# NVlabs/STEP

Hardware: AMD Instinct MI355X
Metric: clips_per_sec_T32_224 (higher is better)
Workload: dtype bf16; 1 GPU; C2: I3D backbone (BaseNet conv3d_1a..mixed_4f) forward, 8 x [3,32,224,224] clips per GPU, inputs resident in HBM, random-init weights; clips_per_gpu=8, T=32, HW=224, parallelism=clip-sharded replicas x1 (no data-path collective), batches_in_flight=2

## Files before the change

step_amd/csrc/common.h:

```cpp
#pragma once
#include <stdint.h>
#include <float.h>
#include <math.h>

#ifdef STEP_EMUL
#include "hipemu.h"
#define STEP_WAVES_PER_SIMD(n)
#define STEP_WAVES_PER_SIMD_MIN(n)
#define STEP_SCHED_BARRIER()
#else
#include <hip/hip_runtime.h>
#define STEP_WAVES_PER_SIMD(n) __attribute__((amdgpu_waves_per_eu(n, n)))
#define STEP_WAVES_PER_SIMD_MIN(n) __attribute__((amdgpu_waves_per_eu(n)))
#define STEP_SCHED_BARRIER() __builtin_amdgcn_sched_barrier(0)
#endif

#include "../../include/step_amd.h"

namespace step {

typedef unsigned short u16x8 __attribute__((ext_vector_type(8)));
typedef unsigned short u16x4 __attribute__((ext_vector_type(4)));
typedef float f32x16 __attribute__((ext_vector_type(16)));
typedef float f32x8 __attribute__((ext_vector_type(8)));
typedef float f32x4 __attribute__((ext_vector_type(4)));
typedef float f32x2 __attribute__((ext_vector_type(2)));
typedef unsigned int u32x4 __attribute__((ext_vector_type(4)));

struct bf16_t { unsigned short v; };
struct f16_t { unsigned short v; };

__device__ __forceinline__ float bf16_bits_to_f32(unsigned short h) {
    unsigned int u = ((unsigned int)h) << 16;
    return __builtin_bit_cast(float, u);
}
__device__ __forceinline__ unsigned short f32_to_bf16_bits(float f) {
#ifndef STEP_EMUL
    return __builtin_bit_cast(unsigned short, (__bf16)f);
#endif
    unsigned int u = __builtin_bit_cast(unsigned int, f);
    if ((u & 0x7fffffffu) > 0x7f800000u) return (unsigned short)((u >> 16) | 0x40);
    u += 0x7fffu + ((u >> 16) & 1u);
    return (unsigned short)(u >> 16);
}
__device__ __forceinline__ float f16_bits_to_f32(unsigned short h) {
    _Float16 x = __builtin_bit_cast(_Float16, h);
    return (float)x;
}
__device__ __forceinline__ unsigned short f32_to_f16_bits(float f) {
    _Float16 x = (_Float16)f;
    return __builtin_bit_cast(unsigned short, x);
}

template <typename T> struct elem;
template <> struct elem<float> {
    static constexpr int dtype = STEP_F32;
    static constexpr int VEC = 4;
    __device__ static __forceinline__ float to_f32(float x) { return x; }
    __device__ static __forceinline__ float from_f32(float x) { return x; }
    __device__ static __forceinline__ unsigned short bits16(float) { return 0; }
    __device__ static __forceinline__ float from_bits16(unsigned short) { return 0.f; }
};
template <> struct elem<bf16_t> {
    static constexpr int dtype = STEP_BF16;
    static constexpr int VEC = 8;
    __device__ static __forceinline__ float to_f32(bf16_t x) { return bf16_bits_to_f32(x.v); }
    __device__ static __forceinline__ bf16_t from_f32(float x) { bf16_t r; r.v = f32_to_bf16_bits(x); return r; }
    __device__ static __forceinline__ unsigned short bits16(float x) { return f32_to_bf16_bits(x); }
    __device__ static __forceinline__ float from_bits16(unsigned short h) { return bf16_bits_to_f32(h); }
};
template <> struct elem<f16_t> {
    static constexpr int dtype = STEP_F16;
    static constexpr int VEC = 8;
    __device__ static __forceinline__ float to_f32(f16_t x) { return f16_bits_to_f32(x.v); }
    __device__ static __forceinline__ f16_t from_f32(float x) { f16_t r; r.v = f32_to_f16_bits(x); return r; }
    __device__ static __forceinline__ unsigned short bits16(float x) { return f32_to_f16_bits(x); }
    __device__ static __forceinline__ float from_bits16(unsigned short h) { return f16_bits_to_f32(h); }
};

template <typename T> struct frag;
template <> struct frag<float> { typedef f32x8 type; };
template <> struct frag<bf16_t> { typedef u16x8 type; };
template <> struct frag<f16_t> { typedef u16x8 type; };

#ifndef STEP_EMUL
typedef __bf16 bf16x8_hw __attribute__((ext_vector_type(8)));
typedef _Float16 f16x8_hw __attribute__((ext_vector_type(8)));
__device__ __forceinline__ void mma_k16(const f32x8& a, const f32x8& b, f32x16& c, float) {
#pragma unroll
    for (int j = 0; j < 8; ++j) c = __builtin_amdgcn_mfma_f32_32x32x2f32(a[j], b[j], c, 0, 0, 0);
}
__device__ __forceinline__ void mma_k16(const u16x8& a, const u16x8& b, f32x16& c, bf16_t) {
    c = __builtin_amdgcn_mfma_f32_32x32x16_bf16(__builtin_bit_cast(bf16x8_hw, a), __builtin_bit_cast(bf16x8_hw, b), c, 0, 0, 0);
}
__device__ __forceinline__ void mma_k16(const u16x8& a, const u16x8& b, f32x16& c, f16_t) {
    c = __builtin_amdgcn_mfma_f32_32x32x16_f16(__builtin_bit_cast(f16x8_hw, a), __builtin_bit_cast(f16x8_hw, b), c, 0, 0, 0);
}
#else
__device__ inline void mma_k16(const f32x8& a, const f32x8& b, f32x16& c, float) {
    float fa[8], fb[8];
    for (int j = 0; j < 8; ++j) { fa[j] = a[j]; fb[j] = b[j]; }
    hipemu::mfma_32x32_k16(fa, fb, c,  true);
}
__device__ inline void mma_k16(const u16x8& a, const u16x8& b, f32x16& c, bf16_t) {
    float fa[8], fb[8];
    for (int j = 0; j < 8; ++j) { fa[j] = bf16_bits_to_f32(a[j]); fb[j] = bf16_bits_to_f32(b[j]); }
    hipemu::mfma_32x32_k16(fa, fb, c, false);
}
__device__ inline void mma_k16(const u16x8& a, const u16x8& b, f32x16& c, f16_t) {
    float fa[8], fb[8];
    for (int j = 0; j < 8; ++j) { fa[j] = f16_bits_to_f32(a[j]); fb[j] = f16_bits_to_f32(b[j]); }
    hipemu::mfma_32x32_k16(fa, fb, c, false);
}
#endif

#ifndef STEP_EMUL
typedef short i16x4_hw __attribute__((ext_vector_type(4)));
__device__ __forceinline__ u16x8 lds_tr8(const unsigned char* a0, const unsigned char* a1) {
    typedef __attribute__((address_space(3))) i16x4_hw* lptr;
    const i16x4_hw lo = __builtin_amdgcn_ds_read_tr16_b64_v4i16((lptr)(const __attribute__((address_space(3))) unsigned char*)a0);
    const i16x4_hw hi = __builtin_amdgcn_ds_read_tr16_b64_v4i16((lptr)(const __attribute__((address_space(3))) unsigned char*)a1);
    u16x8 r = {(unsigned short)lo[0], (unsigned short)lo[1], (unsigned short)lo[2], (unsigned short)lo[3],
               (unsigned short)hi[0], (unsigned short)hi[1], (unsigned short)hi[2], (unsigned short)hi[3]};
    return r;
}
__device__ __forceinline__ void mma16_k32(const u16x8& a, const u16x8& b, f32x4& c, bf16_t) {
    c = __builtin_amdgcn_mfma_f32_16x16x32_bf16(__builtin_bit_cast(bf16x8_hw, a), __builtin_bit_cast(bf16x8_hw, b), c, 0, 0, 0);
}
__device__ __forceinline__ void mma16_k32(const u16x8& a, const u16x8& b, f32x4& c, f16_t) {
    c = __builtin_amdgcn_mfma_f32_16x16x32_f16(__builtin_bit_cast(f16x8_hw, a), __builtin_bit_cast(f16x8_hw, b), c, 0, 0, 0);
}
#else
__device__ inline u16x8 lds_tr8(const unsigned char* a0, const unsigned char* a1) {
    u16x8 r;
    for (int h = 0; h < 2; ++h) {
        unsigned short mine[4], out[4];
        __builtin_memcpy(mine, h ? a1 : a0, 8);
        hipemu::tr16_b64(mine, out);
        for (int j = 0; j < 4; ++j) r[h * 4 + j] = out[j];
    }
    return r;
}
__device__ inline void mma16_k32(const u16x8& a, const u16x8& b, f32x4& c, bf16_t) {
    float fa[8], fb[8];
    for (int j = 0; j < 8; ++j) { fa[j] = bf16_bits_to_f32(a[j]); fb[j] = bf16_bits_to_f32(b[j]); }
    hipemu::mfma_16x16_k32(fa, fb, c);
}
__device__ inline void mma16_k32(const u16x8& a, const u16x8& b, f32x4& c, f16_t) {
    float fa[8], fb[8];
    for (int j = 0; j < 8; ++j) { fa[j] = f16_bits_to_f32(a[j]); fb[j] = f16_bits_to_f32(b[j]); }
    hipemu::mfma_16x16_k32(fa, fb, c);
}
#endif

#ifndef STEP_EMUL
__device__ __forceinline__ void glds16(const void* gsrc_lane, void* lds_base_uniform) {
    __builtin_amdgcn_global_load_lds((const __attribute__((address_space(1))) void*)gsrc_lane,
                                     (__attribute__((address_space(3))) void*)lds_base_uniform, 16, 0, 0);
}
#else
__device__ inline void glds16(const void* gsrc_lane, void* lds_base_uniform) {
    __builtin_memcpy((unsigned char*)lds_base_uniform + 16 * (threadIdx.x & 63), gsrc_lane, 16);
}
#endif

__device__ __forceinline__ int cd_row(int r, int lane) { return (r & 3) + 8 * (r >> 2) + 4 * (lane >> 5); }

#ifndef STEP_EMUL
__device__ __forceinline__ void lane32_swap(unsigned& x, unsigned& y) {
    const auto r = __builtin_amdgcn_permlane32_swap(x, y, false, false);
    x = r[0]; y = r[1];
}
#else
__device__ inline void lane32_swap(unsigned& x, unsigned& y) {
    const unsigned mine[2] = {x, y};
    const int lane = (int)(threadIdx.x & 63);
    char* s = hipemu::exchange_begin(mine, 8);
    unsigned nx = x, ny = y;
    if (lane >= 32) __builtin_memcpy(&nx, s + 256 * (lane - 32) + 4, 4);
    else __builtin_memcpy(&ny, s + 256 * (lane + 32), 4);
    hipemu::exchange_end();
    x = nx; y = ny;
}
#endif

#ifdef STEP_EMUL
#define STEP_LAUNCH(kernel, grid, block, stream, ...) \
    hipemu::launch((grid), (block), [=]() { kernel(__VA_ARGS__); })
#define STEP_LAUNCH_CHECK() 0
#else
#define STEP_LAUNCH(kernel, grid, block, stream, ...) \
    hipLaunchKernelGGL(kernel, (grid), (block), 0, (hipStream_t)(stream), __VA_ARGS__)
#define STEP_LAUNCH_CHECK() ((int)hipGetLastError())
#endif

static inline int ceil_div(int a, int b) { return (a + b - 1) / b; }
static inline long long ceil_div64(long long a, long long b) { return (a + b - 1) / b; }

}
```

step_amd/csrc/stem.hip:

```cpp
#include "conv_common.h"

namespace step {

constexpr int STEM_TH = 8, STEM_TW = 16;
constexpr int STEM_ROWS = 2 * STEM_TH + 5, STEM_COLS = 40;

struct StemParams {
    const void* x; const void* w; const float* scale; const float* shift; void* y;
    int N, T, H, W, To, Ho, Wo, Cout, y_cstride, y_coff;
    int tiles_h, tiles_w, nblk32;
    int tile0;
    int relu;
    int Hp, Wp;
    void* rowbuf;
    void* colbuf;
    int u8_scale; float u8_mean[3], u8_std[3];
#ifdef STEP_PROBE
    unsigned long long* probe;
#endif
};

template <typename T, int NB>
__global__ __launch_bounds__(256) void stem_igemm_kernel(StemParams p) {
    constexpr int ES = (int)sizeof(T);
    constexpr int PIXB = 4 * ES;
    constexpr int NPIX = 7 * STEM_ROWS * STEM_COLS;
    typedef typename frag<T>::type frag_t;
    __shared__ __attribute__((aligned(16))) unsigned char lds[NPIX * PIXB];

    const int tid = threadIdx.x;
    const int lane = tid & 63, wave = tid >> 6;
    const int khalf = lane >> 5;
    const int m = wave * 32 + (lane & 31);
    const int th = m >> 4, tw = m & 15;

    int t = blockIdx.x;
    const int tw_i = t % p.tiles_w; t /= p.tiles_w;
    const int th_i = t % p.tiles_h; t /= p.tiles_h;
    const int od = t % p.To;
    const int n = t / p.To;
    const int oh0 = th_i * STEM_TH, ow0 = tw_i * STEM_TW;
    const int nb0 = blockIdx.y * NB;

    const T* xg = (const T*)p.x;
    const bool vec_ok = (p.W % 4) == 0;
    for (int item = tid; item < 7 * STEM_ROWS * (STEM_COLS / 4); item += 256) {
        const int cq = item % (STEM_COLS / 4);
        const int r = (item / (STEM_COLS / 4)) % STEM_ROWS;
        const int f = item / ((STEM_COLS / 4) * STEM_ROWS);
        const int it = 2 * od - 2 + f, ih = 2 * oh0 - 2 + r, iw0 = 2 * ow0 - 4 + cq * 4;
        T px[4][4];
#pragma unroll
        for (int a = 0; a < 4; ++a)
#pragma unroll
            for (int c = 0; c < 4; ++c) px[a][c] = elem<T>::from_f32(0.f);
        if (it >= 0 && it < p.T && ih >= 0 && ih < p.H) {
            const size_t base = (((size_t)n * p.T + it) * 3) * p.H * p.W + (size_t)ih * p.W;
#pragma unroll
            for (int c = 0; c < 3; ++c) {
                const T* src = xg + base + (size_t)c * p.H * p.W;
                if (vec_ok && iw0 >= 0 && iw0 + 3 < p.W) {
                    typedef unsigned int uvec __attribute__((ext_vector_type(ES)));
                    uvec raw = *(const uvec*)(src + iw0);
                    T v4[4];
                    __builtin_memcpy(v4, &raw, sizeof(v4));
#pragma unroll
                    for (int a = 0; a < 4; ++a) px[a][c] = v4[a];
                } else {
#pragma unroll
                    for (int a = 0; a < 4; ++a)
                        if (iw0 + a >= 0 && iw0 + a < p.W) px[a][c] = src[iw0 + a];
                }
            }
        }
        unsigned char* dst = lds + ((f * STEM_ROWS + r) * STEM_COLS + cq * 4) * PIXB;
#pragma unroll
        for (int q = 0; q < (4 * PIXB) / 16; ++q) {
            u32x4 tmp;
            __builtin_memcpy(&tmp, (const unsigned char*)&px[0][0] + 16 * q, 16);
            *(u32x4*)(dst + 16 * q) = tmp;
        }
    }
    __syncthreads();

    f32x16 acc[NB];
#pragma unroll
    for (int i = 0; i < NB; ++i)
#pragma unroll
        for (int r = 0; r < 16; ++r) acc[i][r] = 0.f;

    const T* wg = (const T*)p.w;
#pragma unroll 1
    for (int kd = 0; kd < 7; ++kd) {
#pragma unroll 1
        for (int kh = 0; kh < 7; ++kh) {
            const unsigned char* rowb = lds + ((kd * STEM_ROWS + 2 * th + kh) * STEM_COLS + 2 * tw + 2) * PIXB;
#pragma unroll
            for (int j = 0; j < 2; ++j) {
                const unsigned char* ap = rowb + (4 * j + 2 * khalf) * PIXB;
                frag_t a;
                {
                    u32x4 h2[ES / 2];
#pragma unroll
                    for (int q = 0; q < ES / 2; ++q) h2[q] = *(const u32x4*)(ap + 16 * q);
                    __builtin_memcpy(&a, h2, sizeof(a));
                }
                const int ks = (kd * 7 + kh) * 2 + j;
#pragma unroll
                for (int i = 0; i < NB; ++i) {
                    if (nb0 + i < p.nblk32) {
                        const T* bp = wg + (((size_t)(nb0 + i) * 98 + ks) * 64 + lane) * 8;
                        const frag_t b = load_b_frag<T>(bp);
                        mma_k16(a, b, acc[i], T());
                    }
                }
            }
        }
    }

    T* yg = (T*)p.y;
#pragma unroll
    for (int i = 0; i < NB; ++i) {
        const int co = (nb0 + i) * 32 + (lane & 31);
        if (nb0 + i < p.nblk32 && co < p.Cout) {
            const float sc = p.scale ? p.scale[co] : 1.f;
            const float sh = p.shift ? p.shift[co] : 0.f;
#pragma unroll
            for (int r = 0; r < 16; ++r) {
                const int mm = wave * 32 + cd_row(r, lane);
                const int oh = oh0 + (mm >> 4), ow = ow0 + (mm & 15);
                if (oh < p.Ho && ow < p.Wo) {
                    float v = acc[i][r] * sc + sh;
                    if (p.relu) v = fmaxf(v, 0.f);
                    const size_t opix = (((size_t)n * p.To + od) * p.Ho + oh) * p.Wo + ow;
                    yg[opix * p.y_cstride + p.y_coff + co] = elem<T>::from_f32(v);
                }
            }
        }
    }
}

constexpr int STP_ROWS = 37, STP_COLS = 40;

constexpr int STS_PITCH = 240;
constexpr int STS_FRAME = STP_ROWS * STS_PITCH;
constexpr int STS_KSTEPS = 77;

__device__ __forceinline__ u16x8 lds_read_frag_a4(const unsigned char* p) {
    typedef unsigned int u32x2_a4 __attribute__((ext_vector_type(2), aligned(4)));
    const u32x2_a4 lo = *(const u32x2_a4*)p;
    const u32x2_a4 hi = *(const u32x2_a4*)(p + 8);
    const u32x4 v = {lo.x, lo.y, hi.x, hi.y};
    u16x8 r;
    __builtin_memcpy(&r, &v, 16);
    return r;
}

constexpr int STS_TPITCH = 144;
typedef short s16x8_t __attribute__((ext_vector_type(8)));
__device__ __forceinline__ u32x4 pk_max_nonneg16(const u32x4& a, const u32x4& b) {
    return __builtin_bit_cast(u32x4, __builtin_elementwise_max(__builtin_bit_cast(s16x8_t, a), __builtin_bit_cast(s16x8_t, b)));
}

template <typename T, int NB_ = 2, bool VEC = true, bool POOL = false, bool U8 = false>
__global__ __launch_bounds__(256) STEP_WAVES_PER_SIMD(3) void stem_stream_kernel(StemParams p) {
    static_assert(sizeof(T) == 2, "16-bit storage types only");
    static_assert(!U8 || VEC, "uint8 frames: whole 4-column quads only");
    constexpr int FRAME = STS_FRAME, PITCH = STS_PITCH;
    constexpr int NB = NB_, FRAGB = 1024;
    constexpr int NBREG = 4 * FRAGB;
    constexpr int BBUF = NB * NBREG;
    constexpr int ITEMS = STP_ROWS * (STP_COLS / 4);
    constexpr int SL = 128;
    constexpr int FQ = (ITEMS + SL - 1) / SL;
    constexpr int NTILES = 21;
    typedef u16x8 frag_t;

    static_assert(!POOL || (NB == 2 && 256 * STS_TPITCH <= 3 * FRAME + 3 * BBUF), "the pooled epilogue's tile lives in the frame / weight rings");
    __shared__ __attribute__((aligned(16))) unsigned char lds[3 * FRAME + 3 * BBUF + NB * 32 * 2 * 4 + (U8 ? 3 * 256 * 2 : 0)];
    unsigned char* const ldsA = lds;
    unsigned char* const ldsB = lds + 3 * FRAME;
    float* const ldsS = (float*)(lds + 3 * FRAME + 3 * BBUF);
    unsigned short* const ldsL = (unsigned short*)(lds + 3 * FRAME + 3 * BBUF + NB * 32 * 2 * 4);

    const int tid = threadIdx.x;
    const int lane = tid & 63;
#ifdef STEP_EMUL
    const int wave = tid >> 6;
#else
    const int wave = __builtin_amdgcn_readfirstlane(tid >> 6);
#endif
    const int khalf = lane >> 5;
    const bool isW = wave < 2;
    const int stid = tid & (SL - 1);

    STEP_PROBE_IDS(p);
    STEP_PROBE_MARK(p, 0);
    int t = blockIdx.x;
    if ((gridDim.x & 7) == 0) t = (t & 7) * (gridDim.x >> 3) + (t >> 3);
    t += p.tile0;
    const int tw_i = t % p.tiles_w; t /= p.tiles_w;
    const int th_i = t % p.tiles_h; t /= p.tiles_h;
    const int od = t % p.To;
    const int n = t / p.To;
    const int oh0 = th_i * 16, ow0 = tw_i * 16;
    const int nb0 = blockIdx.y * NB;

    const T* xg = (const T*)p.x;
    const unsigned char* wg = (const unsigned char*)p.w;
    constexpr bool vec_ok = VEC;

    struct ItemP { u16x4 c[3]; };
    struct ItemB { unsigned w[3]; };
    typedef typename std::conditional<U8, ItemB, ItemP>::type Item;
    int qoff[FQ];
#pragma unroll
    for (int q = 0; q < FQ; ++q) {
        const int item = stid + q * SL;
        const int cq = item % (STP_COLS / 4), r = item / (STP_COLS / 4);
        const int ih = 2 * oh0 - 2 + r, iw0 = 2 * ow0 - 4 + cq * 4;
        qoff[q] = (item < ITEMS && ih >= 0 && ih < p.H && iw0 >= 0 && iw0 + 3 < p.W) ? ih * p.W + iw0 : -1;
    }
    const size_t plane_elems = (size_t)p.H * p.W;
    auto load_frame = [&](int f, Item (&it)[FQ]) {
        const int ifr = 2 * od - 2 + f;
        const bool frok = ifr >= 0 && ifr < p.T;
        const unsigned short* fbase = (const unsigned short*)xg + ((size_t)n * p.T + (frok ? ifr : 0)) * 3 * plane_elems;
        if constexpr (U8) {
            const unsigned char* fb8 = (const unsigned char*)p.x + ((size_t)n * p.T + (frok ? ifr : 0)) * 3 * plane_elems;
#pragma unroll
            for (int q = 0; q < FQ; ++q) {
                const unsigned* src = (const unsigned*)(fb8 + (size_t)(qoff[q] >= 0 ? qoff[q] : 0) * 3);
                it[q].w[0] = src[0]; it[q].w[1] = src[1]; it[q].w[2] = src[2];
            }
        } else if constexpr (vec_ok) {
#pragma unroll
            for (int q = 0; q < FQ; ++q) {
                const unsigned short* src = fbase + (qoff[q] >= 0 ? qoff[q] : 0);
#pragma unroll
                for (int c = 0; c < 3; ++c) it[q].c[c] = *(const u16x4*)(src + c * plane_elems);
            }
        } else {
#pragma unroll
        for (int q = 0; q < FQ; ++q) {
            const int item = stid + q * SL;
            const int cq = item % (STP_COLS / 4), r = item / (STP_COLS / 4);
            const int ih = 2 * oh0 - 2 + r, iw0 = 2 * ow0 - 4 + cq * 4;
            const bool rowok = item < ITEMS && frok && ih >= 0 && ih < p.H;
#pragma unroll
            for (int c = 0; c < 3; ++c) {
                u16x4 v = {0, 0, 0, 0};
                if (rowok) {
                    const unsigned short* src = fbase + c * plane_elems + (size_t)ih * p.W;
#pragma unroll
                    for (int a = 0; a < 4; ++a)
                        if (iw0 + a >= 0 && iw0 + a < p.W) v[a] = src[iw0 + a];
                }
                it[q].c[c] = v;
            }
        }
        }
    };
    auto store_frame = [&](int slotoff, int f, const Item (&it)[FQ]) {
        const int ifr = 2 * od - 2 + f;
        const bool frok = ifr >= 0 && ifr < p.T;
#pragma unroll
        for (int q = 0; q < FQ; ++q) {
            const int item = stid + q * SL;
            if (item < ITEMS) {
                const int cq = item % (STP_COLS / 4), r = item / (STP_COLS / 4);
                unsigned char* dst = ldsA + slotoff + r * PITCH + cq * 24;
                const unsigned short keep = (!vec_ok || (frok && qoff[q] >= 0)) ? 0xffffu : 0u;
                u16x4 v0, v1, v2;
                if constexpr (U8) {
                    unsigned short val[12];
#pragma unroll
                    for (int e = 0; e < 12; ++e) val[e] = ldsL[(e % 3) * 256 + ((it[q].w[e >> 2] >> (8 * (e & 3))) & 0xffu)];
                    v0 = u16x4{val[0], val[1], val[2], val[3]}; v1 = u16x4{val[4], val[5], val[6], val[7]}; v2 = u16x4{val[8], val[9], val[10], val[11]};
                } else {
                    v0 = u16x4{it[q].c[0][0], it[q].c[1][0], it[q].c[2][0], it[q].c[0][1]};
                    v1 = u16x4{it[q].c[1][1], it[q].c[2][1], it[q].c[0][2], it[q].c[1][2]};
                    v2 = u16x4{it[q].c[2][2], it[q].c[0][3], it[q].c[1][3], it[q].c[2][3]};
                }
#pragma unroll
                for (int e = 0; e < 4; ++e) { v0[e] &= keep; v1[e] &= keep; v2[e] &= keep; }
                *(u16x4*)dst = v0;
                *(u16x4*)(dst + 8) = v1;
                *(u16x4*)(dst + 16) = v2;
            }
        }
    };

    const unsigned char* wthr[NB];
#pragma unroll
    for (int i = 0; i < NB; ++i)
        wthr[i] = wg + ((size_t)min(nb0 + i, p.nblk32 - 1) * STS_KSTEPS) * FRAGB + stid * 16;
    struct BReg { u32x4 v[NB][2]; };
    auto load_B = [&](int tile) {
        tile = min(tile, NTILES - 1);
        const int ks0 = (tile / 3) * 11 + (tile % 3) * 4;
        BReg r;
#pragma unroll
        for (int i = 0; i < NB; ++i)
#pragma unroll
            for (int j = 0; j < 2; ++j) r.v[i][j] = *(const u32x4*)(wthr[i] + (size_t)ks0 * FRAGB + j * (SL * 16));
        return r;
    };
    auto store_B = [&](int buf, const BReg& r) {
#pragma unroll
        for (int i = 0; i < NB; ++i)
#pragma unroll
            for (int j = 0; j < 2; ++j) *(u32x4*)(ldsB + buf * BBUF + i * NBREG + j * (SL * 16) + stid * 16) = r.v[i][j];
    };

    const unsigned char* abase[2];
#pragma unroll
    for (int mb = 0; mb < 2; ++mb) {
        const int th = wave * 4 + mb + 2 * ((lane & 31) >> 4), tw = lane & 15;
        abase[mb] = ldsA + (2 * th) * PITCH + (2 * tw + 2) * 6;
    }
    const int kh_row = khalf * PITCH, kh_q = khalf * 16;
    const unsigned char* const bwave = ldsB + lane * 16;

    f32x16 acc[2][NB];
#pragma unroll
    for (int mb = 0; mb < 2; ++mb)
#pragma unroll
        for (int i = 0; i < NB; ++i)
#pragma unroll
            for (int r = 0; r < 16; ++r) acc[mb][i][r] = 0.f;

    frag_t fa[2][2], fb[2][NB];
    auto read_frags = [&](auto setc, auto jc, int slotoff) {
        constexpr int SET = decltype(setc)::value;
        constexpr int J = decltype(jc)::value;
        const int aoff = slotoff + (J < 9 ? (2 * (J / 3)) * PITCH + (J % 3) * 16 + kh_row : (J == 9 ? 6 * PITCH + kh_q : 6 * PITCH + 32));
#pragma unroll
        for (int mb = 0; mb < 2; ++mb) fa[SET][mb] = lds_read_frag_a4(abase[mb] + aoff);
#pragma unroll
        for (int i = 0; i < NB; ++i) fb[SET][i] = *(const frag_t*)(bwave + (J / 4) * BBUF + i * NBREG + (J % 4) * FRAGB);
    };
    auto mma_all = [&](auto setc) {
        constexpr int SET = decltype(setc)::value;
#pragma unroll
        for (int i = 0; i < NB; ++i) {
            mma_k16(fb[SET][i], fa[SET][0], acc[0][i], T());
            mma_k16(fb[SET][i], fa[SET][1], acc[1][i], T());
        }
    };

    if constexpr (U8) {
#pragma unroll
        for (int k = 0; k < 3; ++k) {
            float v = (float)tid;
            if (p.u8_scale == 1) v = __fdiv_rn(v, 255.f);
            else if (p.u8_scale == 2) v = __fsub_rn(__fdiv_rn(__fmul_rn(v, 2.f), 255.f), 1.f);
            v = __fdiv_rn(__fsub_rn(v, p.u8_mean[k]), p.u8_std[k]);
            ldsL[k * 256 + tid] = elem<T>::bits16(v);
        }
        __syncthreads();
    }
    auto run_role = [&](auto rolec) {
    constexpr bool W = decltype(rolec)::value;
    Item fr[FQ], fr1[FQ];
    Item frS[FQ];
    BReg R, R1;
    if constexpr (W) {
        float ss_sc = 1.f, ss_sh = 0.f;
        R = load_B(0);
        R1 = load_B(1);
        if (tid < NB * 32) {
            const int co = min(nb0 * 32 + tid, p.Cout - 1);
            if (p.scale) ss_sc = p.scale[co];
            if (p.shift) ss_sh = p.shift[co];
        }
        store_B(0, R);
        store_B(1, R1);
        if (tid < NB * 32) { ldsS[tid] = ss_sc; ldsS[NB * 32 + tid] = ss_sh; }
        R = load_B(2);
    } else {
        load_frame(0, fr);
        load_frame(1, fr1);
        load_frame(2, frS);
        store_frame(0, 0, fr);
        store_frame(FRAME, 1, fr1);
    }
    __syncthreads();
    STEP_PROBE_MARK(p, 1);
    read_frags(std::integral_constant<int, 0>(), std::integral_constant<int, 0>(), 0);

    int cur = 0, nxt = FRAME, nn = 2 * FRAME;
    auto frame_iter = [&](auto pc, auto ldc, auto stc, int kd) {
        constexpr int P = decltype(pc)::value;
        constexpr bool LD = decltype(ldc)::value, ST = decltype(stc)::value;
#define STS_KSTEP(J)                                                                                                  \
        {                                                                                                             \
            if (J < 10) read_frags(std::integral_constant<int, (P + J + 1) & 1>(), std::integral_constant<int, (J + 1) % 11>(), cur); \
            else        read_frags(std::integral_constant<int, (P + J + 1) & 1>(), std::integral_constant<int, 0>(), nxt);            \
            mma_all(std::integral_constant<int, (P + J) & 1>());                                                      \
        }
#define STS_TILE_END(TI)                                                                                              \
        {                                                                                                             \
            if constexpr (W) {                                                                                        \
                store_B((TI + 2) % 3, R);                                \
                R = load_B(3 * kd + TI + 3);                                                                          \
            }                                                                                                         \
        }
        STS_KSTEP(0) STS_KSTEP(1) STS_KSTEP(2) STS_KSTEP(3)
        STS_TILE_END(0)
        __syncthreads();
        STS_KSTEP(4) STS_KSTEP(5) STS_KSTEP(6) STS_KSTEP(7)
        STS_TILE_END(1)
        if constexpr (ST && !W) {
            STEP_SCHED_BARRIER();
            store_frame(nn, kd + 2, frS);
            if constexpr (LD) load_frame(kd + 3, frS);
        }
        __syncthreads();
        STS_KSTEP(8) STS_KSTEP(9) STS_KSTEP(10)
        STS_TILE_END(2)
        __syncthreads();
#undef STS_KSTEP
#undef STS_TILE_END
        const int tmp = cur; cur = nxt; nxt = nn; nn = tmp;
    };
#pragma unroll 1
    for (int kd = 0; kd < 4; kd += 2) {
        frame_iter(std::integral_constant<int, 0>(), std::true_type(), std::true_type(), kd);
        frame_iter(std::integral_constant<int, 1>(), std::true_type(), std::true_type(), kd + 1);
        STEP_PROBE_MARK(p, 5 + kd / 2);
    }
    frame_iter(std::integral_constant<int, 0>(), std::false_type(), std::true_type(), 4);
    frame_iter(std::integral_constant<int, 1>(), std::false_type(), std::false_type(), 5);
    STEP_PROBE_MARK(p, 7);
    frame_iter(std::integral_constant<int, 0>(), std::false_type(), std::false_type(), 6);
    };
    if (isW) run_role(std::true_type());
    else run_role(std::false_type());
    STEP_PROBE_MARK(p, 2);

    T* yg = (T*)p.y;
    const bool vec_epi = (p.y_cstride % 8 == 0) && (p.y_coff % 8 == 0) && (p.Cout % 8 == 0) && (((uintptr_t)p.y) % 16 == 0);
#pragma unroll
    for (int mb = 0; mb < 2; ++mb) {
        const int oh = oh0 + wave * 4 + mb + 2 * ((lane & 31) >> 4), ow = ow0 + (lane & 15);
        const bool okp = oh < p.Ho && ow < p.Wo;
        const size_t opix = okp ? (((size_t)n * p.To + od) * p.Ho + oh) * p.Wo + ow : 0;
#pragma unroll
        for (int i = 0; i < NB; ++i) {
            unsigned d[4][2];
#pragma unroll
            for (int g = 0; g < 4; ++g) {
                const f32x4 sc = *(const f32x4*)(ldsS + i * 32 + 8 * g + 4 * khalf);
                const f32x4 sh = *(const f32x4*)(ldsS + NB * 32 + i * 32 + 8 * g + 4 * khalf);
                float v[4];
#pragma unroll
                for (int e = 0; e < 4; ++e) {
                    v[e] = acc[mb][i][4 * g + e] * sc[e] + sh[e];
                    if (p.relu) v[e] = fmaxf(v[e], 0.f);
                }
                if (!vec_epi && !POOL) {
#pragma unroll
                    for (int e = 0; e < 4; ++e) {
                        const int co = (nb0 + i) * 32 + 8 * g + 4 * khalf + e;
                        if (okp && co < p.Cout) yg[opix * p.y_cstride + p.y_coff + co] = elem<T>::from_f32(v[e]);
                    }
                }
                d[g][0] = (unsigned)elem<T>::bits16(v[0]) | ((unsigned)elem<T>::bits16(v[1]) << 16);
                d[g][1] = (unsigned)elem<T>::bits16(v[2]) | ((unsigned)elem<T>::bits16(v[3]) << 16);
            }
            if constexpr (POOL) {
                const int tpix = (wave * 4 + mb + 2 * ((lane & 31) >> 4)) * 16 + (lane & 15);
#pragma unroll
                for (int h = 0; h < 2; ++h) {
                    lane32_swap(d[2 * h][0], d[2 * h + 1][0]);
                    lane32_swap(d[2 * h][1], d[2 * h + 1][1]);
                    u32x4 o = {d[2 * h][0], d[2 * h][1], d[2 * h + 1][0], d[2 * h + 1][1]};
                    if (!okp) o = u32x4{0u, 0u, 0u, 0u};
                    *(u32x4*)(lds + tpix * STS_TPITCH + (i * 32 + 16 * h + 8 * khalf) * 2) = o;
                }
            } else if (vec_epi) {
#pragma unroll
                for (int h = 0; h < 2; ++h) {
                    lane32_swap(d[2 * h][0], d[2 * h + 1][0]);
                    lane32_swap(d[2 * h][1], d[2 * h + 1][1]);
                    const int co = (nb0 + i) * 32 + 16 * h + 8 * khalf;
                    if (okp && co < p.Cout) {
                        const u32x4 o = {d[2 * h][0], d[2 * h][1], d[2 * h + 1][0], d[2 * h + 1][1]};
                        *(u32x4*)(yg + opix * p.y_cstride + p.y_coff + co) = o;
                    }
                }
            }
        }
    }
    if constexpr (POOL) {
        __syncthreads();
        const size_t plane = (size_t)n * p.To + od;
#pragma unroll
        for (int k = 0; k < 2; ++k) {
            const int item = tid + 256 * k;
            const int v = item & 7, q = (item >> 3) & 7, j = item >> 6;
            const unsigned char* base = lds + ((2 * j) * 16 + 2 * q) * STS_TPITCH + v * 16;
            u32x4 m = *(const u32x4*)base;
#pragma unroll
            for (int dr = 0; dr < 3; ++dr)
#pragma unroll
                for (int dc = 0; dc < 3; ++dc) {
                    if (dr == 0 && dc == 0) continue;
                    if (2 * j + dr < 16 && 2 * q + dc < 16) m = pk_max_nonneg16(m, *(const u32x4*)(base + (dr * 16 + dc) * STS_TPITCH));
                }
            const int ph = (oh0 >> 1) + j, pw = (ow0 >> 1) + q;
            if (ph < p.Hp && pw < p.Wp)
                *(u32x4*)(yg + ((plane * p.Hp + ph) * p.Wp + pw) * p.y_cstride + p.y_coff + v * 8) = m;
        }
        {
            const int v = tid & 7, e = (tid >> 3) & 15;
            unsigned short* rb = (unsigned short*)p.rowbuf;
            unsigned short* cb = (unsigned short*)p.colbuf;
            if (tid < 128) {
                if (th_i > 0 && ow0 + e < p.Wo)
                    *(u32x4*)(rb + ((plane * p.tiles_h + th_i) * p.Wo + ow0 + e) * (size_t)p.Cout + v * 8) = *(const u32x4*)(lds + e * STS_TPITCH + v * 16);
            } else {
                if (tw_i > 0 && oh0 + e < p.Ho)
                    *(u32x4*)(cb + ((plane * p.tiles_w + tw_i) * p.Ho + oh0 + e) * (size_t)p.Cout + v * 8) = *(const u32x4*)(lds + (e * 16) * STS_TPITCH + v * 16);
            }
        }
    }
#ifdef STEP_PROBE
    STEP_PROBE_MARK(p, 3);
    __builtin_amdgcn_s_waitcnt(0);
    probe_clock_end(p.probe);
    STEP_PROBE_MARK(p, 4);
#endif
}

__global__ __launch_bounds__(256) void stem_pool_fix_kernel(StemParams p) {
    const int nbr = p.tiles_h - 1, nbc = p.tiles_w - 1;
    const long long per_plane = ((long long)nbr * p.Wp + (long long)nbc * p.Hp) * (p.Cout / 8);
    const long long total = per_plane * p.N * p.To;
    const int V = p.Cout / 8;
    unsigned short* yg = (unsigned short*)p.y;
    const unsigned short* rb = (const unsigned short*)p.rowbuf;
    const unsigned short* cb = (const unsigned short*)p.colbuf;
    for (long long idx = (long long)blockIdx.x * blockDim.x + threadIdx.x; idx < total; idx += (long long)blockDim.x * gridDim.x) {
        const long long plane = idx / per_plane;
        long long it = idx % per_plane;
        const int v = (int)(it % V);
        it /= V;
        int ph, pw;
        bool row_item;
        if (it < (long long)nbr * p.Wp) { row_item = true; ph = 8 * ((int)(it / p.Wp) + 1) - 1; pw = (int)(it % p.Wp); }
        else { it -= (long long)nbr * p.Wp; row_item = false; pw = 8 * ((int)(it / p.Hp) + 1) - 1; ph = (int)(it % p.Hp); }
        if (ph >= p.Hp || pw >= p.Wp) continue;
        const bool ph_seam = ((ph + 1) & 7) == 0 && ((ph + 1) >> 3) <= nbr;
        const bool pw_seam = ((pw + 1) & 7) == 0 && ((pw + 1) >> 3) <= nbc;
        if (!row_item && ph_seam) continue;
        unsigned short* yp = yg + ((plane * p.Hp + ph) * p.Wp + pw) * (size_t)p.y_cstride + p.y_coff + v * 8;
        u32x4 m = *(const u32x4*)yp;
        if (row_item) {
            const int t = (ph + 1) >> 3;
            for (int dc = 0; dc < 3; ++dc) {
                const int c = 2 * pw + dc;
                if (c < p.Wo) m = pk_max_nonneg16(m, *(const u32x4*)(rb + ((plane * p.tiles_h + t) * p.Wo + c) * (size_t)p.Cout + v * 8));
            }
            if (pw_seam) {
                const int s = (pw + 1) >> 3;
                for (int dr = 0; dr < 2; ++dr)
                    m = pk_max_nonneg16(m, *(const u32x4*)(cb + ((plane * p.tiles_w + s) * p.Ho + 2 * ph + dr) * (size_t)p.Cout + v * 8));
            }
        } else {
            const int s = (pw + 1) >> 3;
            for (int dr = 0; dr < 3; ++dr) {
                const int r = 2 * ph + dr;
                if (r < p.Ho) m = pk_max_nonneg16(m, *(const u32x4*)(cb + ((plane * p.tiles_w + s) * p.Ho + r) * (size_t)p.Cout + v * 8));
            }
        }
        *(u32x4*)yp = m;
    }
}

template <typename T>
__global__ void stem_stream_pack_weight_kernel(const float* __restrict__ w, T* __restrict__ out, int Cout, long long total) {
    for (long long idx = (long long)blockIdx.x * blockDim.x + threadIdx.x; idx < total;
         idx += (long long)blockDim.x * gridDim.x) {
        const int e = (int)(idx & 7);
        const int lane = (int)((idx >> 3) & 63);
        const long long q = idx >> 9;
        const int ks = (int)(q % STS_KSTEPS);
        const long long nb = q / STS_KSTEPS;
        const int kd = ks / 11, j = ks % 11, khalf = lane >> 5;
        int kh, fq;
        if (j < 9) { kh = 2 * (j / 3) + khalf; fq = j % 3; }
        else if (j == 9) { kh = 6; fq = khalf; }
        else { kh = 6; fq = khalf ? -1 : 2; }
        const int se = 8 * fq + e, kw = se / 3, c = se % 3;
        const long long co = nb * 32 + (lane & 31);
        float v = 0.f;
        if (fq >= 0 && co < Cout && kw < 7) v = w[((((size_t)co * 3 + c) * 7 + kd) * 7 + kh) * 7 + kw];
        out[idx] = elem<T>::from_f32(v);
    }
}

template <typename T>
__global__ void stem_pack_weight_kernel(const float* __restrict__ w, T* __restrict__ out, int Cout, long long total) {
    for (long long idx = (long long)blockIdx.x * blockDim.x + threadIdx.x; idx < total;
         idx += (long long)blockDim.x * gridDim.x) {
        const int e = (int)(idx & 7);
        const int lane = (int)((idx >> 3) & 63);
        long long q = idx >> 9;
        const int ks = (int)(q % 98);
        const int nb = (int)(q / 98);
        const int j = ks & 1, kh = (ks >> 1) % 7, kd = (ks >> 1) / 7;
        const int kw = 4 * j + 2 * (lane >> 5) + (e >> 2), c = e & 3;
        const int co = nb * 32 + (lane & 31);
        float v = 0.f;
        if (co < Cout && c < 3 && kw < 7) v = w[((((size_t)co * 3 + c) * 7 + kd) * 7 + kh) * 7 + kw];
        out[idx] = elem<T>::from_f32(v);
    }
}


template <typename T>
static int stem_forward_t(StemParams p, step_stream_t stream) {
    dim3 grid((unsigned)((long long)p.N * p.To * p.tiles_h * p.tiles_w), (unsigned)ceil_div(p.nblk32, 2));
    STEP_LAUNCH((stem_igemm_kernel<T, 2>), grid, dim3(256), stream, p);
    return STEP_LAUNCH_CHECK();
}

static inline size_t stem_stream_offset(int Cout) { return (size_t)ceil_div(Cout, 32) * 98 * 512; }

template <typename T>
static int stem_stream_forward_t(StemParams p, step_stream_t stream) {
    p.w = (const T*)p.w + stem_stream_offset(p.Cout);
    p.tiles_h = ceil_div(p.Ho, 16); p.tiles_w = ceil_div(p.Wo, 16);
    const long long tiles = (long long)p.N * p.To * p.tiles_h * p.tiles_w;
    const int groups = ceil_div(p.nblk32, 2);
    p.tile0 = 0;
#ifdef STEP_PROBE
    p.probe = g_probe_buf;
#endif
    dim3 grid((unsigned)tiles, (unsigned)groups);
    if (p.W % 4 == 0) STEP_LAUNCH((stem_stream_kernel<T, 2, true>), grid, dim3(256), stream, p);
    else STEP_LAUNCH((stem_stream_kernel<T, 2, false>), grid, dim3(256), stream, p);
    return STEP_LAUNCH_CHECK();
}


}

using namespace step;

extern "C" {

size_t step_stem_packed_elems(int Cout) { return stem_stream_offset(Cout) + ((size_t)ceil_div(Cout, 32) * STS_KSTEPS + 1) * 512; }

int step_stem_pack_weight(const float* w, int Cout, int dtype, void* packed, step_stream_t stream) {
    if (Cout <= 0) return STEP_E_SHAPE;
    if (!w || !packed) return STEP_E_NULL;
    const long long total = (long long)stem_stream_offset(Cout);
    const long long total2 = (long long)step_stem_packed_elems(Cout) - total;
    const dim3 grid(flat_grid(total, 256)), grid2(flat_grid(total2, 256));
    switch (dtype) {
        case STEP_F32:
            STEP_LAUNCH((stem_pack_weight_kernel<float>), grid, dim3(256), stream, w, (float*)packed, Cout, total);
            STEP_LAUNCH((stem_stream_pack_weight_kernel<float>), grid2, dim3(256), stream, w, (float*)packed + total, Cout, total2);
            break;
        case STEP_BF16:
            STEP_LAUNCH((stem_pack_weight_kernel<bf16_t>), grid, dim3(256), stream, w, (bf16_t*)packed, Cout, total);
            STEP_LAUNCH((stem_stream_pack_weight_kernel<bf16_t>), grid2, dim3(256), stream, w, (bf16_t*)packed + total, Cout, total2);
            break;
        case STEP_F16:
            STEP_LAUNCH((stem_pack_weight_kernel<f16_t>), grid, dim3(256), stream, w, (f16_t*)packed, Cout, total);
            STEP_LAUNCH((stem_stream_pack_weight_kernel<f16_t>), grid2, dim3(256), stream, w, (f16_t*)packed + total, Cout, total2);
            break;
        default: return STEP_E_DTYPE;
    }
    return STEP_LAUNCH_CHECK();
}

int step_stem_forward(int dtype, const void* x, int N, int T, int H, int W, const void* w_packed, const float* scale,
                      const float* shift, int relu, int Cout, void* y, int y_cstride, int y_coff, step_stream_t stream) {
    if (N < 0 || T <= 0 || H <= 0 || W <= 0 || Cout <= 0) return STEP_E_SHAPE;
    if (y_coff < 0 || y_coff + Cout > y_cstride) return STEP_E_SHAPE;
    if (N == 0) return STEP_OK;
    if (!x || !w_packed || !y) return STEP_E_NULL;
    if (((uintptr_t)x % 16) || ((uintptr_t)w_packed % 16)) return STEP_E_ALIGN;
    StemParams p;
    p.x = x; p.w = w_packed; p.scale = scale; p.shift = shift; p.y = y;
    p.N = N; p.T = T; p.H = H; p.W = W; p.tile0 = 0; p.relu = relu != 0;
    p.To = (T + 5 - 7) / 2 + 1; p.Ho = (H + 5 - 7) / 2 + 1; p.Wo = (W + 5 - 7) / 2 + 1;
    if (p.To <= 0 || p.Ho <= 0 || p.Wo <= 0) return STEP_E_SHAPE;
    p.Cout = Cout; p.y_cstride = y_cstride; p.y_coff = y_coff;
    p.tiles_h = ceil_div(p.Ho, STEM_TH); p.tiles_w = ceil_div(p.Wo, STEM_TW);
    p.nblk32 = ceil_div(Cout, 32);
    const int ov = conv_impl_override();
    switch (dtype) {
        case STEP_F32: return stem_forward_t<float>(p, stream);
        case STEP_BF16: return ov == 0 ? stem_forward_t<bf16_t>(p, stream) : stem_stream_forward_t<bf16_t>(p, stream);
        case STEP_F16: return ov == 0 ? stem_forward_t<f16_t>(p, stream) : stem_stream_forward_t<f16_t>(p, stream);
    }
    return STEP_E_DTYPE;
}


static bool stem_pool_supported(int dtype, int N, int T, int H, int W, int Cout) {
    return (dtype == STEP_BF16 || dtype == STEP_F16) && N > 0 && T > 0 && H > 0 && W > 0 && (W % 4) == 0 && Cout == 64 && conv_impl_override() != 0;
}

size_t step_stem_pool_workspace_bytes(int dtype, int N, int T, int H, int W, int Cout) {
    if (!stem_pool_supported(dtype, N, T, H, W, Cout)) return 0;
    const int To = (T - 2) / 2 + 1, Ho = (H - 2) / 2 + 1, Wo = (W - 2) / 2 + 1;
    const size_t planes = (size_t)N * To;
    return planes * ((size_t)ceil_div(Ho, 16) * Wo + (size_t)ceil_div(Wo, 16) * Ho) * Cout * 2 + 32;
}

static int stem_pool_forward_impl(int dtype, const void* x, int N, int T, int H, int W, const void* w_packed, const float* scale, const float* shift,
                                  int Cout, void* y, int y_cstride, int y_coff, void* ws, size_t ws_bytes, int parts, step_stream_t stream) {
    if (N < 0 || T <= 0 || H <= 0 || W <= 0 || Cout <= 0) return STEP_E_SHAPE;
    if (y_coff < 0 || y_coff + Cout > y_cstride) return STEP_E_SHAPE;
    if (N == 0) return STEP_OK;
    if (!stem_pool_supported(dtype, N, T, H, W, Cout)) return STEP_E_UNSUPPORTED;
    if (!x || !w_packed || !y || !ws) return STEP_E_NULL;
    if (((uintptr_t)x % 16) || ((uintptr_t)w_packed % 16) || ((uintptr_t)y % 16) || ((uintptr_t)ws % 16) || (y_cstride % 8) || (y_coff % 8)) return STEP_E_ALIGN;
    if (ws_bytes < step_stem_pool_workspace_bytes(dtype, N, T, H, W, Cout)) return STEP_E_SHAPE;
    StemParams p;
    p.x = x; p.scale = scale; p.shift = shift; p.y = y;
    p.N = N; p.T = T; p.H = H; p.W = W; p.tile0 = 0; p.relu = 1;
    p.To = (T + 5 - 7) / 2 + 1; p.Ho = (H + 5 - 7) / 2 + 1; p.Wo = (W + 5 - 7) / 2 + 1;
    if (p.To <= 0 || p.Ho <= 0 || p.Wo <= 0) return STEP_E_SHAPE;
    p.Cout = Cout; p.y_cstride = y_cstride; p.y_coff = y_coff;
    p.nblk32 = ceil_div(Cout, 32);
    p.tiles_h = ceil_div(p.Ho, 16); p.tiles_w = ceil_div(p.Wo, 16);
    p.Hp = step_pool_out_size(p.Ho, 3, 2); p.Wp = step_pool_out_size(p.Wo, 3, 2);
    p.rowbuf = ws;
    p.colbuf = (unsigned char*)ws + (((size_t)N * p.To * p.tiles_h * p.Wo * Cout * 2 + 15) / 16) * 16;
#ifdef STEP_PROBE
    p.probe = g_probe_buf;
#endif
    const long long tiles = (long long)p.N * p.To * p.tiles_h * p.tiles_w;
    dim3 grid((unsigned)tiles, 1);
    if (parts & 1) {
        if (dtype == STEP_BF16) {
            p.w = (const bf16_t*)w_packed + stem_stream_offset(Cout);
            STEP_LAUNCH((stem_stream_kernel<bf16_t, 2, true, true>), grid, dim3(256), stream, p);
        } else {
            p.w = (const f16_t*)w_packed + stem_stream_offset(Cout);
            STEP_LAUNCH((stem_stream_kernel<f16_t, 2, true, true>), grid, dim3(256), stream, p);
        }
    }
    if ((parts & 2) && (p.tiles_h > 1 || p.tiles_w > 1)) {
        const long long items = ((long long)(p.tiles_h - 1) * p.Wp + (long long)(p.tiles_w - 1) * p.Hp) * (Cout / 8) * p.N * p.To;
        STEP_LAUNCH(stem_pool_fix_kernel, dim3(flat_grid(items, 256)), dim3(256), stream, p);
    }
    return STEP_LAUNCH_CHECK();
}

int step_stem_pool_forward(int dtype, const void* x, int N, int T, int H, int W, const void* w_packed, const float* scale, const float* shift,
                           int Cout, void* y, int y_cstride, int y_coff, void* ws, size_t ws_bytes, step_stream_t stream) {
    return stem_pool_forward_impl(dtype, x, N, T, H, W, w_packed, scale, shift, Cout, y, y_cstride, y_coff, ws, ws_bytes, 3, stream);
}

int step_stem_pool_forward_tiles(int dtype, const void* x, int N, int T, int H, int W, const void* w_packed, const float* scale, const float* shift,
                                 int Cout, void* y, int y_cstride, int y_coff, void* ws, size_t ws_bytes, step_stream_t stream) {
    return stem_pool_forward_impl(dtype, x, N, T, H, W, w_packed, scale, shift, Cout, y, y_cstride, y_coff, ws, ws_bytes, 1, stream);
}

int step_stem_pool_finish(int dtype, const void* x, int N, int T, int H, int W, int Cout, void* y, int y_cstride, int y_coff, void* ws, size_t ws_bytes,
                          step_stream_t stream) {
    return stem_pool_forward_impl(dtype, x, N, T, H, W, x, nullptr, nullptr, Cout, y, y_cstride, y_coff, ws, ws_bytes, 2, stream);
}

int step_stem_pool_forward_u8(int dtype, const unsigned char* frames, int N, int T, int H, int W, int u8_scale, const float* mean3, const float* std3,
                              const void* w_packed, const float* scale, const float* shift, int Cout, void* y, int y_cstride, int y_coff,
                              void* ws, size_t ws_bytes, step_stream_t stream) {
    if (N < 0 || T <= 0 || H <= 0 || W <= 0 || Cout <= 0 || u8_scale < 0 || u8_scale > 2) return STEP_E_SHAPE;
    if (y_coff < 0 || y_coff + Cout > y_cstride) return STEP_E_SHAPE;
    if (N == 0) return STEP_OK;
    if (!stem_pool_supported(dtype, N, T, H, W, Cout)) return STEP_E_UNSUPPORTED;
    if (!frames || !w_packed || !y || !ws) return STEP_E_NULL;
    if (((uintptr_t)frames % 4) || ((uintptr_t)w_packed % 16) || ((uintptr_t)y % 16) || ((uintptr_t)ws % 16) || (y_cstride % 8) || (y_coff % 8)) return STEP_E_ALIGN;
    if (ws_bytes < step_stem_pool_workspace_bytes(dtype, N, T, H, W, Cout)) return STEP_E_SHAPE;
    StemParams p;
    p.x = frames; p.scale = scale; p.shift = shift; p.y = y;
    p.N = N; p.T = T; p.H = H; p.W = W; p.tile0 = 0; p.relu = 1;
    p.To = (T + 5 - 7) / 2 + 1; p.Ho = (H + 5 - 7) / 2 + 1; p.Wo = (W + 5 - 7) / 2 + 1;
    if (p.To <= 0 || p.Ho <= 0 || p.Wo <= 0) return STEP_E_SHAPE;
    p.Cout = Cout; p.y_cstride = y_cstride; p.y_coff = y_coff;
    p.nblk32 = ceil_div(Cout, 32);
    p.tiles_h = ceil_div(p.Ho, 16); p.tiles_w = ceil_div(p.Wo, 16);
    p.Hp = step_pool_out_size(p.Ho, 3, 2); p.Wp = step_pool_out_size(p.Wo, 3, 2);
    p.rowbuf = ws;
    p.colbuf = (unsigned char*)ws + (((size_t)N * p.To * p.tiles_h * p.Wo * Cout * 2 + 15) / 16) * 16;
    p.u8_scale = u8_scale;
    for (int c = 0; c < 3; ++c) { p.u8_mean[c] = mean3 ? mean3[c] : 0.f; p.u8_std[c] = std3 ? std3[c] : 1.f; }
#ifdef STEP_PROBE
    p.probe = g_probe_buf;
#endif
    const long long tiles = (long long)p.N * p.To * p.tiles_h * p.tiles_w;
    dim3 grid((unsigned)tiles, 1);
    if (dtype == STEP_BF16) {
        p.w = (const bf16_t*)w_packed + stem_stream_offset(Cout);
        STEP_LAUNCH((stem_stream_kernel<bf16_t, 2, true, true, true>), grid, dim3(256), stream, p);
    } else {
        p.w = (const f16_t*)w_packed + stem_stream_offset(Cout);
        STEP_LAUNCH((stem_stream_kernel<f16_t, 2, true, true, true>), grid, dim3(256), stream, p);
    }
    if (p.tiles_h > 1 || p.tiles_w > 1) {
        const long long items = ((long long)(p.tiles_h - 1) * p.Wp + (long long)(p.tiles_w - 1) * p.Hp) * (Cout / 8) * p.N * p.To;
        STEP_LAUNCH(stem_pool_fix_kernel, dim3(flat_grid(items, 256)), dim3(256), stream, p);
    }
    return STEP_LAUNCH_CHECK();
}

int step_stem_kernel_name(int dtype, char* buf, int buflen) {
    if (!buf || buflen <= 0) return STEP_E_NULL;
    const int ov = conv_impl_override();
    const char* t = dtype == STEP_F32 ? "float" : (dtype == STEP_BF16 ? "step::bf16_t" : "step::f16_t");
    if (dtype != STEP_F32 && dtype != STEP_BF16 && dtype != STEP_F16) return STEP_E_DTYPE;
    if (dtype == STEP_F32 || ov == 0) snprintf(buf, (size_t)buflen, "void step::stem_igemm_kernel<%s, 2>(step::StemParams)", t);
    else snprintf(buf, (size_t)buflen, "void step::stem_stream_kernel<%s, 2, true, false, false>(step::StemParams)", t);
    return STEP_OK;
}


}
```

Before: 7552 clips/s.

## Stream stem weight tiles via direct global-to-LDS DMA with four-deep ring

The weight waves of the stem conv kernel now load weight fragments with global_load_lds straight into LDS instead of going through registers and storing them. Each tile shrinks from four k-steps to three, and the ring grows to four buffers, giving 28 tiles with a vmcnt-based wait. An extra barrier per frame separates the new fourth tile. The intent is to remove VGPR staging and LDS store instructions on the weight path and keep more weight loads in flight. In exchange it uses more LDS, adds one __syncthreads per frame, and relies on hand-written m0 asm whose vmcnt accounting must match exactly.

```diff
diff --git a/step_amd/csrc/common.h b/step_amd/csrc/common.h
--- a/step_amd/csrc/common.h
+++ b/step_amd/csrc/common.h
@@ -164,6 +164,19 @@
 }
 #endif
 
+#ifndef STEP_EMUL
+__device__ __forceinline__ void glds16_uncounted(const void* gsrc_lane, void* lds_base_uniform) {
+    const unsigned dst = __builtin_amdgcn_readfirstlane((unsigned)(uintptr_t)(__attribute__((address_space(3))) void*)lds_base_uniform);
+    unsigned keep;
+    asm volatile("s_mov_b32 %0, m0\n\ts_mov_b32 m0, %2\n\ts_nop 0\n\tglobal_load_lds_dwordx4 %1, off\n\ts_mov_b32 m0, %0"
+                 : "=&s"(keep) : "v"(gsrc_lane), "s"(dst) : "memory");
+}
+template <int N> __device__ __forceinline__ void vmcnt_wait() { asm volatile("s_waitcnt vmcnt(%0)" :: "i"(N) : "memory"); }
+#else
+__device__ inline void glds16_uncounted(const void* gsrc_lane, void* lds_base_uniform) { glds16(gsrc_lane, lds_base_uniform); }
+template <int N> __device__ inline void vmcnt_wait() {}
+#endif
+
 __device__ __forceinline__ int cd_row(int r, int lane) { return (r & 3) + 8 * (r >> 2) + 4 * (lane >> 5); }
 
 #ifndef STEP_EMUL
diff --git a/step_amd/csrc/stem.hip b/step_amd/csrc/stem.hip
--- a/step_amd/csrc/stem.hip
+++ b/step_amd/csrc/stem.hip
@@ -168,20 +168,22 @@
     static_assert(!U8 || VEC, "uint8 frames: whole 4-column quads only");
     constexpr int FRAME = STS_FRAME, PITCH = STS_PITCH;
     constexpr int NB = NB_, FRAGB = 1024;
-    constexpr int NBREG = 4 * FRAGB;
+    constexpr int NBREG = 3 * FRAGB;
     constexpr int BBUF = NB * NBREG;
+    constexpr int WPW = NB * 3 / 2;
     constexpr int ITEMS = STP_ROWS * (STP_COLS / 4);
     constexpr int SL = 128;
     constexpr int FQ = (ITEMS + SL - 1) / SL;
-    constexpr int NTILES = 21;
+    constexpr int NTILES = 28;
+    static_assert(NB * 3 % 2 == 0, "a tile's weight pieces split evenly over the two weight waves");
     typedef u16x8 frag_t;
 
-    static_assert(!POOL || (NB == 2 && 256 * STS_TPITCH <= 3 * FRAME + 3 * BBUF), "the pooled epilogue's tile lives in the frame / weight rings");
-    __shared__ __attribute__((aligned(16))) unsigned char lds[3 * FRAME + 3 * BBUF + NB * 32 * 2 * 4 + (U8 ? 3 * 256 * 2 : 0)];
+    static_assert(!POOL || (NB == 2 && 256 * STS_TPITCH <= 3 * FRAME + 4 * BBUF), "the pooled epilogue's tile lives in the frame / weight rings");
+    __shared__ __attribute__((aligned(16))) unsigned char lds[3 * FRAME + 4 * BBUF + NB * 32 * 2 * 4 + (U8 ? 3 * 256 * 2 : 0)];
     unsigned char* const ldsA = lds;
     unsigned char* const ldsB = lds + 3 * FRAME;
-    float* const ldsS = (float*)(lds + 3 * FRAME + 3 * BBUF);
-    unsigned short* const ldsL = (unsigned short*)(lds + 3 * FRAME + 3 * BBUF + NB * 32 * 2 * 4);
+    float* const ldsS = (float*)(lds + 3 * FRAME + 4 * BBUF);
+    unsigned short* const ldsL = (unsigned short*)(lds + 3 * FRAME + 4 * BBUF + NB * 32 * 2 * 4);
 
     const int tid = threadIdx.x;
     const int lane = tid & 63;
@@ -294,23 +296,16 @@
     const unsigned char* wthr[NB];
 #pragma unroll
     for (int i = 0; i < NB; ++i)
-        wthr[i] = wg + ((size_t)min(nb0 + i, p.nblk32 - 1) * STS_KSTEPS) * FRAGB + stid * 16;
-    struct BReg { u32x4 v[NB][2]; };
-    auto load_B = [&](int tile) {
-        tile = min(tile, NTILES - 1);
-        const int ks0 = (tile / 3) * 11 + (tile % 3) * 4;
-        BReg r;
-#pragma unroll
-        for (int i = 0; i < NB; ++i)
-#pragma unroll
-            for (int j = 0; j < 2; ++j) r.v[i][j] = *(const u32x4*)(wthr[i] + (size_t)ks0 * FRAGB + j * (SL * 16));
-        return r;
-    };
-    auto store_B = [&](int buf, const BReg& r) {
-#pragma unroll
-        for (int i = 0; i < NB; ++i)
-#pragma unroll
-            for (int j = 0; j < 2; ++j) *(u32x4*)(ldsB + buf * BBUF + i * NBREG + j * (SL * 16) + stid * 16) = r.v[i][j];
+        wthr[i] = wg + ((size_t)min(nb0 + i, p.nblk32 - 1) * STS_KSTEPS) * FRAGB + lane * 16;
+    auto dma_B = [&](int tile) {
+        if (tile >= NTILES) return;
+        const int ks0 = (tile / 4) * 11 + (tile % 4) * 3;
+        unsigned char* const dst = ldsB + (tile % 4) * BBUF;
+#pragma unroll
+        for (int m = 0; m < WPW; ++m) {
+            const int pc = wave + 2 * m, i = pc / 3, k = pc % 3;
+            glds16_uncounted(wthr[i] + (size_t)(ks0 + k) * FRAGB, dst + i * NBREG + k * FRAGB);
+        }
     };
 
     const unsigned char* abase[2];
@@ -338,7 +333,7 @@
 #pragma unroll
         for (int mb = 0; mb < 2; ++mb) fa[SET][mb] = lds_read_frag_a4(abase[mb] + aoff);
 #pragma unroll
-        for (int i = 0; i < NB; ++i) fb[SET][i] = *(const frag_t*)(bwave + (J / 4) * BBUF + i * NBREG + (J % 4) * FRAGB);
+        for (int i = 0; i < NB; ++i) fb[SET][i] = *(const frag_t*)(bwave + (J / 3) * BBUF + i * NBREG + (J % 3) * FRAGB);
     };
     auto mma_all = [&](auto setc) {
         constexpr int SET = decltype(setc)::value;
@@ -364,20 +359,18 @@
     constexpr bool W = decltype(rolec)::value;
     Item fr[FQ], fr1[FQ];
     Item frS[FQ];
-    BReg R, R1;
     if constexpr (W) {
         float ss_sc = 1.f, ss_sh = 0.f;
-        R = load_B(0);
-        R1 = load_B(1);
+        dma_B(0);
+        dma_B(1);
+        dma_B(2);
         if (tid < NB * 32) {
             const int co = min(nb0 * 32 + tid, p.Cout - 1);
             if (p.scale) ss_sc = p.scale[co];
             if (p.shift) ss_sh = p.shift[co];
         }
-        store_B(0, R);
-        store_B(1, R1);
         if (tid < NB * 32) { ldsS[tid] = ss_sc; ldsS[NB * 32 + tid] = ss_sh; }
-        R = load_B(2);
+        vmcnt_wait<WPW>();
     } else {
         load_frame(0, fr);
         load_frame(1, fr1);
@@ -399,17 +392,23 @@
             else        read_frags(std::integral_constant<int, (P + J + 1) & 1>(), std::integral_constant<int, 0>(), nxt);            \
             mma_all(std::integral_constant<int, (P + J) & 1>());                                                      \
         }
+#define STS_TILE_START(TI)                                                                                            \
+        {                                                                                                             \
+            if constexpr (W) dma_B(4 * kd + TI + 3);                   \
+        }
 #define STS_TILE_END(TI)                                                                                              \
         {                                                                                                             \
-            if constexpr (W) {                                                                                        \
-                store_B((TI + 2) % 3, R);                                \
-                R = load_B(3 * kd + TI + 3);                                                                          \
+            if constexpr (W) {                          \
+                if (4 * kd + TI + 3 < NTILES) vmcnt_wait<WPW>();                                                      \
+                else vmcnt_wait<0>();                                                                                 \
             }                                                                                                         \
         }
-        STS_KSTEP(0) STS_KSTEP(1) STS_KSTEP(2) STS_KSTEP(3)
+        STS_TILE_START(0)
+        STS_KSTEP(0) STS_KSTEP(1) STS_KSTEP(2)
         STS_TILE_END(0)
         __syncthreads();
-        STS_KSTEP(4) STS_KSTEP(5) STS_KSTEP(6) STS_KSTEP(7)
+        STS_TILE_START(1)
+        STS_KSTEP(3) STS_KSTEP(4) STS_KSTEP(5)
         STS_TILE_END(1)
         if constexpr (ST && !W) {
             STEP_SCHED_BARRIER();
@@ -417,10 +416,16 @@
             if constexpr (LD) load_frame(kd + 3, frS);
         }
         __syncthreads();
-        STS_KSTEP(8) STS_KSTEP(9) STS_KSTEP(10)
+        STS_TILE_START(2)
+        STS_KSTEP(6) STS_KSTEP(7) STS_KSTEP(8)
         STS_TILE_END(2)
         __syncthreads();
+        STS_TILE_START(3)
+        STS_KSTEP(9) STS_KSTEP(10)
+        STS_TILE_END(3)
+        __syncthreads();
 #undef STS_KSTEP
+#undef STS_TILE_START
 #undef STS_TILE_END
         const int tmp = cur; cur = nxt; nxt = nn; nn = tmp;
     };
```

After: 7560 clips/s (median of 6 runs). About the same (+0.1%).
